# libnxz/power-gzip

Measured on AMD Instinct MI355X. Metric: GiB/s uncompressed in (deflate), real-data corpus in 64 KiB blocks, exact dynamic-Huffman table per block, higher is better.
Workload: dtype u8

## Files before the change

power-gzip_amd/csrc/nxz_cksum_slices.h:

```cpp
#ifndef NXZ_CKSUM_SLICES_H
#define NXZ_CKSUM_SLICES_H
#include <stdint.h>
#ifdef __HIPCC__
#define NXZ_CK_FN __device__ __forceinline__
#define NXZ_CK_TABLE __device__ const
#define NXZ_CK_GLOBAL __attribute__((address_space(1)))
#define NXZ_CK_UDOT4(a, b, c) __builtin_amdgcn_udot4(a, b, c, false)
#else
#define NXZ_CK_FN inline
#define NXZ_CK_TABLE static const
#define NXZ_CK_GLOBAL
static inline uint32_t nxz_ck_udot4(uint32_t a, uint32_t b, uint32_t c)
{
	for (int k = 0; k < 4; k++) c += ((a >> (8 * k)) & 0xff) * ((b >> (8 * k)) & 0xff);
	return c;
}
#define NXZ_CK_UDOT4(a, b, c) nxz_ck_udot4(a, b, c)
#endif

namespace nxzck {

constexpr uint32_t POLY = 0xedb88320u;
constexpr uint32_t ADLER_MOD = 65521u;
constexpr uint32_t SLICE = 64;
constexpr uint32_t LANES = 256;
constexpr uint32_t PER_LANE = 4;

NXZ_CK_FN uint32_t gf_mul(uint32_t a, uint32_t b)
{
	uint32_t r = 0;
#pragma unroll 8
	for (int i = 0; i < 32; i++) {
		r ^= (b & 0x80000000u) ? a : 0;
		a = (a >> 1) ^ ((a & 1) ? POLY : 0);
		b <<= 1;
	}
	return r;
}

constexpr uint32_t cgf_mul(uint32_t a, uint32_t b)
{
	uint32_t r = 0;
	for (int i = 0; i < 32; i++) {
		if (b & 0x80000000u) r ^= a;
		a = (a >> 1) ^ ((a & 1) ? POLY : 0);
		b <<= 1;
	}
	return r;
}
struct PowTab { uint32_t v[1024]; };
constexpr PowTab make_pow()
{
	PowTab p{};
	uint32_t m = 0x00800000u;
	for (int k = 0; k < 6; k++) m = cgf_mul(m, m);
	p.v[0] = 0x80000000u;
	for (int i = 1; i < 1024; i++) p.v[i] = cgf_mul(p.v[i - 1], m);
	return p;
}
NXZ_CK_TABLE PowTab CRC_POW = make_pow();
struct Pow8Tab { uint32_t v[65]; };
constexpr Pow8Tab make_pow8()
{
	Pow8Tab p{};
	p.v[0] = 0x80000000u;
	for (int i = 1; i <= 64; i++) p.v[i] = cgf_mul(p.v[i - 1], 0x00800000u);
	return p;
}
NXZ_CK_TABLE Pow8Tab CRC_POW8 = make_pow8();

NXZ_CK_FN void table_column(uint32_t *T, uint32_t i)
{
	uint32_t c = i;
	for (int k = 0; k < 4; k++) {
		for (int b = 0; b < 8; b++) c = (c >> 1) ^ ((c & 1) ? POLY : 0);
		T[k * 256 + i] = c;
	}
}
NXZ_CK_FN uint32_t crc_dword(const uint32_t *T, uint32_t crc, uint32_t w)
{
	const uint32_t c = crc ^ w;
	return T[768 + (c & 0xff)] ^ T[512 + ((c >> 8) & 0xff)] ^ T[256 + ((c >> 16) & 0xff)] ^ T[c >> 24];
}
NXZ_CK_FN uint32_t crc_byte(const uint32_t *T, uint32_t crc, uint32_t b) { return T[(crc ^ b) & 0xff] ^ (crc >> 8); }

struct Shape {
	uint32_t n, K1, r;
};
NXZ_CK_FN Shape shape_of(uint32_t n)
{
	Shape s;
	s.n = n; s.K1 = n ? (n - 1) >> 6 : 0; s.r = n - s.K1 * SLICE;
	return s;
}

struct Part { uint32_t crc, tailcrc, s1, s2; };

typedef uint32_t ck_v4u __attribute__((vector_size(16)));

NXZ_CK_FN void adler_dword(uint32_t w, uint32_t k, uint32_t &S, uint32_t &Wt)
{
	S = NXZ_CK_UDOT4(w, 0x01010101u, S);
	Wt = NXZ_CK_UDOT4(w, 0x03020100u + 0x04040404u * k, Wt);
}

NXZ_CK_FN Part lane_part(const uint8_t *src_, const Shape sh, uint32_t initx, uint32_t lane, const uint32_t *T)
{
	const NXZ_CK_GLOBAL uint8_t *src = (const NXZ_CK_GLOBAL uint8_t *)src_;
	Part p = { 0, 0, 0, 0 };
	if (!sh.n) return p;
#pragma unroll
	for (uint32_t pr = 0; pr < PER_LANE / 2; pr++) {
		const uint32_t j0 = PER_LANE * lane + 2 * pr;
		if (j0 >= sh.K1) break;
		const bool have1 = j0 + 1 < sh.K1;
		ck_v4u v[2][SLICE / 16];
#pragma unroll
		for (uint32_t q = 0; q < SLICE / 16; q++) {
			__builtin_memcpy(&v[0][q], src + (size_t)j0 * SLICE + 16 * q, 16);
			v[1][q] = (ck_v4u){ 0, 0, 0, 0 };
			if (have1) __builtin_memcpy(&v[1][q], src + (size_t)(j0 + 1) * SLICE + 16 * q, 16);
		}
		uint32_t c0 = j0 == 0 ? initx : 0, c1 = 0, S0 = 0, S1 = 0, W0 = 0, W1 = 0;
#pragma unroll
		for (uint32_t k = 0; k < SLICE / 4; k++) {
			const uint32_t w0 = v[0][k >> 2][k & 3], w1 = v[1][k >> 2][k & 3];
			adler_dword(w0, k, S0, W0);
			adler_dword(w1, k, S1, W1);
			c0 = crc_dword(T, c0, w0);
			c1 = crc_dword(T, c1, w1);
		}
		p.crc ^= gf_mul(c0, CRC_POW.v[sh.K1 - 1 - j0]);
		p.s1 += S0;
		p.s2 += (S0 * (sh.n - j0 * SLICE) - W0) % ADLER_MOD;
		if (have1) {
			p.crc ^= gf_mul(c1, CRC_POW.v[sh.K1 - 2 - j0]);
			p.s1 += S1;
			p.s2 += (S1 * (sh.n - (j0 + 1) * SLICE) - W1) % ADLER_MOD;
		}
	}
	if (sh.K1 / PER_LANE == lane) {
		const uint32_t a = sh.K1 * SLICE;
		uint32_t c = sh.K1 == 0 ? initx : 0, St = 0, Wtt = 0;
		const uint32_t nd = sh.r >> 2;
		for (uint32_t k = 0; k < nd; k++) {
			uint32_t w;
			__builtin_memcpy(&w, src + a + 4 * k, 4);
			adler_dword(w, k, St, Wtt);
			c = crc_dword(T, c, w);
		}
		for (uint32_t k = 4 * nd; k < sh.r; k++) {
			const uint32_t b = src[a + k];
			St += b; Wtt += b * k;
			c = crc_byte(T, c, b);
		}
		p.tailcrc = c;
		p.s1 += St;
		p.s2 += (St * sh.r - Wtt) % ADLER_MOD;
	}
	return p;
}

NXZ_CK_FN void finish(const Shape sh, uint32_t in_crc, uint32_t in_adler, uint32_t crc, uint32_t tailcrc, uint32_t s1, uint32_t s2,
		      uint32_t &out_crc, uint32_t &out_adler)
{
	const uint32_t initx = in_crc ^ 0xffffffffu;
	const uint32_t c = sh.n ? gf_mul(crc, CRC_POW8.v[sh.r]) ^ tailcrc : initx;
	const uint32_t ia = in_adler & 0xffff, ib = in_adler >> 16;
	const uint32_t s1f = (ia + s1) % ADLER_MOD;
	const uint32_t s2f = (uint32_t)(((uint64_t)ib + (uint64_t)sh.n * ia + s2) % ADLER_MOD);
	out_crc = c ^ 0xffffffffu;
	out_adler = (s2f << 16) | s1f;
}

}
#endif
```

Measured before the change: 107.4.

## Chain CRC across two slice pairs per lane to cut GF multiplies

Each lane now carries two running CRCs (slices j0,j0+1 and j0+2,j0+3) across both halves instead of restarting per slice. They are combined with one constant multiply by x^1024, done as a shift-xor table, and a single gf_mul by a new shifted power table that covers negative offsets. This replaces up to four variable gf_mul calls per lane with one variable and one constant multiply. The shape also changes so full 64-byte slices are processed and the tail may be empty, which is skipped. The unroll-1 outer loop trades some ILP for smaller code and fewer registers.

```diff
diff --git a/power-gzip_amd/csrc/nxz_cksum_slices.h b/power-gzip_amd/csrc/nxz_cksum_slices.h
--- a/power-gzip_amd/csrc/nxz_cksum_slices.h
+++ b/power-gzip_amd/csrc/nxz_cksum_slices.h
@@ -59,6 +59,35 @@
 	return p;
 }
 NXZ_CK_TABLE PowTab CRC_POW = make_pow();
+constexpr uint32_t cgf_div_x(uint32_t a) { return (a & 0x80000000u) ? (((a ^ POLY) << 1) | 1u) : (a << 1); }
+constexpr PowTab make_pow4()
+{
+	PowTab p{};
+	const uint32_t x512 = make_pow().v[1];
+	uint32_t m = 0x80000000u;
+	for (int i = 0; i < 3 * 512; i++) m = cgf_div_x(m);
+	p.v[0] = m;
+	for (int i = 1; i < 1024; i++) p.v[i] = cgf_mul(p.v[i - 1], x512);
+	return p;
+}
+NXZ_CK_TABLE PowTab CRC_POW4 = make_pow4();
+static_assert(make_pow4().v[3] == 0x80000000u && make_pow4().v[1023] == make_pow().v[1020], "x^-1536 x^1536 = 1");
+constexpr uint32_t X1024 = make_pow().v[2];
+struct MulTab { uint32_t v[32]; };
+constexpr MulTab make_mul(uint32_t c)
+{
+	MulTab m{};
+	for (int i = 0; i < 32; i++) m.v[i] = cgf_mul(c, 1u << i);
+	return m;
+}
+NXZ_CK_FN uint32_t gf_mul_x1024(uint32_t a)
+{
+	constexpr MulTab M = make_mul(X1024);
+	uint32_t r = 0;
+#pragma unroll
+	for (int i = 0; i < 32; i++) r ^= ((a >> i) & 1) ? M.v[i] : 0;
+	return r;
+}
 struct Pow8Tab { uint32_t v[65]; };
 constexpr Pow8Tab make_pow8()
 {
@@ -90,7 +119,7 @@
 NXZ_CK_FN Shape shape_of(uint32_t n)
 {
 	Shape s;
-	s.n = n; s.K1 = n ? (n - 1) >> 6 : 0; s.r = n - s.K1 * SLICE;
+	s.n = n; s.K1 = n >> 6; s.r = n & (SLICE - 1);
 	return s;
 }
 
@@ -109,37 +138,39 @@
 	const NXZ_CK_GLOBAL uint8_t *src = (const NXZ_CK_GLOBAL uint8_t *)src_;
 	Part p = { 0, 0, 0, 0 };
 	if (!sh.n) return p;
-#pragma unroll
-	for (uint32_t pr = 0; pr < PER_LANE / 2; pr++) {
-		const uint32_t j0 = PER_LANE * lane + 2 * pr;
-		if (j0 >= sh.K1) break;
-		const bool have1 = j0 + 1 < sh.K1;
-		ck_v4u v[2][SLICE / 16];
-#pragma unroll
-		for (uint32_t q = 0; q < SLICE / 16; q++) {
-			__builtin_memcpy(&v[0][q], src + (size_t)j0 * SLICE + 16 * q, 16);
-			v[1][q] = (ck_v4u){ 0, 0, 0, 0 };
-			if (have1) __builtin_memcpy(&v[1][q], src + (size_t)(j0 + 1) * SLICE + 16 * q, 16);
+	const uint32_t j0 = PER_LANE * lane;
+	if (j0 < sh.K1) {
+		uint32_t cA = j0 == 0 ? initx : 0, cB = 0;
+#pragma unroll 1
+		for (uint32_t hf = 0; hf < 2; hf++) {
+			const uint32_t jA = j0 + hf, jB = j0 + 2 + hf;
+			const bool haveA = jA < sh.K1, haveB = jB < sh.K1;
+			ck_v4u v[2][SLICE / 16];
+#pragma unroll
+			for (uint32_t q = 0; q < SLICE / 16; q++) v[0][q] = v[1][q] = (ck_v4u){ 0, 0, 0, 0 };
+			if (haveA) {
+#pragma unroll
+				for (uint32_t q = 0; q < SLICE / 16; q++) __builtin_memcpy(&v[0][q], src + (size_t)jA * SLICE + 16 * q, 16);
+			}
+			if (haveB) {
+#pragma unroll
+				for (uint32_t q = 0; q < SLICE / 16; q++) __builtin_memcpy(&v[1][q], src + (size_t)jB * SLICE + 16 * q, 16);
+			}
+			uint32_t SA = 0, SB = 0, WA = 0, WB = 0;
+#pragma unroll
+			for (uint32_t k = 0; k < SLICE / 4; k++) {
+				const uint32_t wA = v[0][k >> 2][k & 3], wB = v[1][k >> 2][k & 3];
+				adler_dword(wA, k, SA, WA);
+				adler_dword(wB, k, SB, WB);
+				cA = crc_dword(T, cA, wA);
+				cB = crc_dword(T, cB, wB);
+			}
+			p.s1 += SA + SB;
+			p.s2 += (SA * (sh.n - jA * SLICE) - WA) % ADLER_MOD + (SB * (sh.n - jB * SLICE) - WB) % ADLER_MOD;
 		}
-		uint32_t c0 = j0 == 0 ? initx : 0, c1 = 0, S0 = 0, S1 = 0, W0 = 0, W1 = 0;
-#pragma unroll
-		for (uint32_t k = 0; k < SLICE / 4; k++) {
-			const uint32_t w0 = v[0][k >> 2][k & 3], w1 = v[1][k >> 2][k & 3];
-			adler_dword(w0, k, S0, W0);
-			adler_dword(w1, k, S1, W1);
-			c0 = crc_dword(T, c0, w0);
-			c1 = crc_dword(T, c1, w1);
-		}
-		p.crc ^= gf_mul(c0, CRC_POW.v[sh.K1 - 1 - j0]);
-		p.s1 += S0;
-		p.s2 += (S0 * (sh.n - j0 * SLICE) - W0) % ADLER_MOD;
-		if (have1) {
-			p.crc ^= gf_mul(c1, CRC_POW.v[sh.K1 - 2 - j0]);
-			p.s1 += S1;
-			p.s2 += (S1 * (sh.n - (j0 + 1) * SLICE) - W1) % ADLER_MOD;
-		}
-	}
-	if (sh.K1 / PER_LANE == lane) {
+		p.crc = gf_mul(gf_mul_x1024(cA) ^ cB, CRC_POW4.v[sh.K1 - j0 - 1]);
+	}
+	if (sh.r && sh.K1 / PER_LANE == lane) {
 		const uint32_t a = sh.K1 * SLICE;
 		uint32_t c = sh.K1 == 0 ? initx : 0, St = 0, Wtt = 0;
 		const uint32_t nd = sh.r >> 2;
```

Result: no change. 108.0 (median of 6 runs) (+0.6%).
